# NyanCAD/Cadnip.jl

Hardware: AMD Instinct MI355X
Metric: newton_iters_per_sec (higher is better)
Workload: dtype f64; 1 GPU; gf180 DFF transient 0-700 ns (synthetic sp_mos1 level-1 card, 30 MOSFETs, n=235, nnz=1090), 4096 Vdd x temp corner instances per GPU (state resident in HBM; one 8-instance workgroup per CU in flight, the rest handed out by the kernel's instance queue); step = DC init + full transient of the batch; instances_per_gpu=4096, instances_total=4096, fused=2, newton_mode=1, launches_last_step=5120, accepted_last_step=6078488, rejected_last_step=692364

## Files before the change

### cadnip.jl_amd/csrc/devices.hpp

```cpp
#pragma once
#include <hip/hip_runtime.h>
#include <math.h>
#include "../../include/cadnip_hip.h"

namespace cadnip {

#define CADNIP_CHARGE_SCALE 1e12

#ifdef CADNIP_TRACE
static __device__ unsigned long long g_trace_sum[64], g_trace_cnt[64];
static __device__ int g_trace_wave;
__shared__ unsigned long long g_trace_last;
#define CADNIP_TRACE_FINE(id) (((id) >= 8 && (id) <= 15) || (id) >= 18 || (id) == 0 || (id) == 2)
#define CADNIP_TRACE_POINT(id)                                                                          \
  do {                                                                                                  \
    if ((CADNIP_TRACE + 0 >= 2 || !CADNIP_TRACE_FINE(id)) && blockIdx.x == 0 && (int)(threadIdx.x >> 6) == g_trace_wave) { \
      unsigned long long _t = clock64();                                                                \
      if ((threadIdx.x & 63) == 0) {                                                                    \
        atomicAdd(&g_trace_sum[id], _t - g_trace_last); atomicAdd(&g_trace_cnt[id], 1ull); g_trace_last = _t; \
      }                                                                                                 \
    }                                                                                                   \
  } while (0)
#define CADNIP_TRACE_USE(x) asm volatile("" ::"v"(x))
#elif defined(CADNIP_MARKS)
// ... 504 lines not shown
      D3 vddif = 2.0 * vdsat - vds, vddif1 = vdsat - vds, vddif2 = vddif * vddif;
      capgd = cox * (1.0 - vdsat * vdsat / vddif2) / 3;
      capgs = cox * (1.0 - vddif1 * vddif1 / vddif2) / 3;
      capgb = D3(0.0);
    }
  }
}

template <bool FQ = true>
__device__ inline D3 m1_qdep(const D3& v, double Cb, double Cbsw, double tBulkPot, double tDepCap, double mj, double mjsw,
                             double f2, double f3, double f4) {
  if (Cb != 0 || Cbsw != 0) {
    if (v.v < tDepCap) {
      D3 arg = 1.0 - m1_over<FQ>(v, tBulkPot);
      D3 sarg = (mj == 0.5) ? m1_recip<FQ>(m1_dsqrt<FQ>(arg)) : dexp(-mj * m1_dlog<FQ>(arg));
      D3 sargsw = (mjsw == mj) ? sarg : ((mjsw == 0.5) ? m1_recip<FQ>(m1_dsqrt<FQ>(arg)) : dexp(-mjsw * m1_dlog<FQ>(arg)));
      return tBulkPot * (m1_over<FQ>(Cb * (1.0 - arg * sarg), 1 - mj) + m1_over<FQ>(Cbsw * (1.0 - arg * sargsw), 1 - mjsw));
    }
    return f4 + v * (f2 + v * (f3 / 2));
  }
  return D3(0.0);
}

template <class Ctx>
__device__ inline void m1_limit(const Ctx& d, const double* u, double type, double vt, double tPhi, double tVbi, double gamma, double Vg, double Vb,
                                double Vdi, double Vsi, int l0, int l1, int l2, int l3, double& w_gs, double& w_ds, double& w_bs, double& w_bd) {
  double o_vgs = type * u[l0], o_vds = type * u[l1], o_vbs = type * u[l2], o_vbd = type * u[l3];
  double vbs = type * (Vb - Vsi), vgs = type * (Vg - Vsi), vds = type * (Vdi - Vsi);
  double vbd = vbs - vds, vgd = vgs - vds, vgdo = o_vgs - o_vds;
  {
    const bool fwd = o_vds >= 0;
    const double q_vgs = fwd ? vgs : vgd + (vgs - vgd), q_vgd = fwd ? vgs - (vgs - vgd) : vgd, q_vds = vgs - vgd;
    const bool c1 = fabs(fwd ? vgs - o_vgs : vgd - vgdo) <= 0.4, c2 = fabs(q_vds - o_vds) <= 0.4;
    const bool c3 = q_vds >= 0 ? !(fabs(vbs - o_vbs) > (vt + vt)) : !(fabs(vbd - o_vbd) > (vt + vt));
    if (__all(c1 && c2 && c3)) {
      double r_vgs = q_vgs, r_vds = q_vds, r_vbs, r_vbd;
      (void)q_vgd;
      if (r_vds >= 0) { r_vbs = vbs; r_vbd = r_vbs - r_vds; }
      else { r_vbd = vbd; r_vbs = r_vbd + r_vds; }
      if (d.initjct) { r_vbs = -1; r_vgs = type * par_of(d, M1_TVTO); r_vds = 0; r_vbd = r_vbs - r_vds; }
      w_gs = type * r_vgs; w_ds = type * r_vds; w_bs = type * r_vbs; w_bd = type * r_vbd;
      return;
    }
  }
  int omode = o_vds >= 0 ? 1 : -1;
  double osel = omode == 1 ? o_vbs : o_vbd, osarg;
  if (osel <= 0) osarg = sqrt(tPhi - osel);
  else { osarg = sqrt(tPhi); osarg = osarg - o_vbs / (osarg + osarg); osarg = fmax(0.0, osarg); }
  double o_von = (tVbi * type) + gamma * osarg;
  double von = type * o_von;
// ... 163 lines not shown
}


__device__ __forceinline__ D3 m1_swap_pair(const D3& x) {
  D3 r;
  r.v = dpp_pair_swap(x.v);
#pragma unroll
  for (int i = 0; i < 3; ++i) r.p[i] = dpp_pair_swap(x.p[i]);
  return r;
}
__device__ __forceinline__ D3 m1_sel(bool c, const D3& x, const D3& y) {
  D3 r;
  r.v = c ? x.v : y.v;
#pragma unroll
  for (int i = 0; i < 3; ++i) r.p[i] = c ? x.p[i] : y.p[i];
  return r;
}


template <class Ctx, class Out>
__device__ inline void stamp_mos1_pair(const Ctx& d, const double* u, const Out& s, double* limit_w_base, int side, bool valid) {
  const double CS = CADNIP_CHARGE_SCALE;
  const bool D = side != 0;
  int nd = node_of(d, 0), ng = node_of(d, 1), ns = node_of(d, 2), nb = node_of(d, 3), ndi = node_of(d, 4), nsi = node_of(d, 5);
  int l0 = node_of(d, 6), l1 = node_of(d, 7), l2 = node_of(d, 8), l3 = node_of(d, 9);
  double Vd = volt(u, nd), Vg = volt(u, ng), Vs = volt(u, ns), Vb = volt(u, nb), Vdi = volt(u, ndi), Vsi = volt(u, nsi);
  double type = par_of(d, M1_TYPE), vt = par_of(d, M1_VT), tPhi = par_of(d, M1_TPHI), tVbi = par_of(d, M1_TVBI);
  double gamma = par_of(d, M1_GAMMA);
  const double mf = par_of(d, M1_MFACTOR), gmin_p = par_of(d, M1_GMIN), isat = par_of(d, D ? M1_DSATCUR : M1_SSATCUR);
  const double lambda = par_of(d, M1_LAMBDA), Beta = par_of(d, M1_BETA);
  const int vdep = Out::DIRECT ? d.ipar[d.dev] : 0;
  __builtin_amdgcn_sched_barrier(0);
  CADNIP_TRACE_USE(Vd); CADNIP_TRACE_USE(Vg); CADNIP_TRACE_USE(Vs); CADNIP_TRACE_USE(Vb); CADNIP_TRACE_USE(Vdi); CADNIP_TRACE_USE(Vsi);
  CADNIP_TRACE_POINT(18);
  CADNIP_TRACE_USE(type);
  CADNIP_TRACE_POINT(19);
  CADNIP_TRACE_POINT(20);
  double w_gs, w_ds, w_bs, w_bd;
  m1_limit(d, u, type, vt, tPhi, tVbi, gamma, Vg, Vb, Vdi, Vsi, l0, l1, l2, l3, w_gs, w_ds, w_bs, w_bd);
  if (limit_w_base && valid && !D) { limit_w_base[l0] = w_gs; limit_w_base[l1] = w_ds; limit_w_base[l2] = w_bs; limit_w_base[l3] = w_bd; }
  CADNIP_TRACE_POINT(21);
  {
    const double gl[6] = {1.0, -1.0, 1.0, 1.0, -1.0, 1.0};
    s.Gv(6 * side, gl);
    if constexpr (Out::DIRECT) {
      s.Rn(D ? l2 : l0, u[D ? l2 : l0] - ((D ? Vb : Vg) - Vsi));
      s.Rn(D ? l3 : l1, u[D ? l3 : l1] - (D ? Vb - Vdi : Vdi - Vsi));
    }
  }
  CADNIP_TRACE_POINT(22);
  D3 a = D3::seed(type * w_gs, 0), b = D3::seed(type * w_ds, 1), c = D3::seed(type * w_bs, 2);
  D3 dvbd = c - b, dvgd = a - b;
  const D3 vj = m1_sel(D, dvbd, c);
  const double gmin_m = fast_div(gmin_p, mf);
  const double q_cb = par_of(d, D ? M1_CBD : M1_CBS), q_cbsw = par_of(d, D ? M1_CBDSW : M1_CBSSW), q_pot = par_of(d, M1_TBULKPOT), q_dep = par_of(d, M1_TDEPCAP);
  const double q_mj = par_of(d, M1_MJ), q_mjsw = par_of(d, M1_MJSW), q_f2 = par_of(d, D ? M1_F2D : M1_F2S), q_f3 = par_of(d, D ? M1_F3D : M1_F3S), q_f4 = par_of(d, D ? M1_F4D : M1_F4S);
  __builtin_amdgcn_sched_barrier(0);
  const D3 cj = m1_junction(vj, vt, gmin_m, isat), co = m1_swap_pair(cj);
  const D3 cbs = m1_sel(D, co, cj), cbd = m1_sel(D, cj, co);
  CADNIP_TRACE_POINT(23);
  int mode;
  D3 dvon, vdsat, cdrain;
  m1_channel(a, b, c, dvbd, dvgd, tPhi, tVbi, type, gamma, lambda, Beta, mode, dvon, vdsat, cdrain);
  CADNIP_TRACE_POINT(24);
  const D3 cdreq = (mode >= 0 ? type : -type) * cdrain;
  const double dW_gs = (Vg - Vsi) - w_gs, dW_ds = (Vdi - Vsi) - w_ds, dW_bs = (Vb - Vsi) - w_bs;
  const double Vk[6] = {Vd, Vg, Vs, Vb, Vdi, Vsi};
  auto row = [&](const D3& I, double (&g)[6], double& Ieq) {
    const double fa = type * I.p[0], fb = type * I.p[1], fc = type * I.p[2];
    g[0] = 0.0; g[1] = mf * fa; g[2] = 0.0; g[3] = mf * fc; g[4] = mf * fb; g[5] = mf * -(fa + fb + fc);
    Ieq = mf * I.v;
#pragma unroll
    for (int k = 0; k < 6; ++k) Ieq = Ieq + (-g[k] * Vk[k]);
    Ieq = Ieq + (mf * type * I.p[0]) * dW_gs;
    Ieq = Ieq + (mf * type * I.p[1]) * dW_ds;
    Ieq = Ieq + (mf * type * I.p[2]) * dW_bs;
  };
  {
    const D3 I3 = type * cbs + type * cbd, I4 = -1.0 * (type * cbd - cdreq);
    double g[6], Ieq;
    row(m1_sel(D, I4, I3), g, Ieq);
    const int br = 3 + side;
    s.Gv(12 + 6 * br, g);
    s.B(br, -Ieq);
    if constexpr (Out::DIRECT) {
      const D3 I = m1_sel(D, I4, I3);
      s.Rn(D ? ndi : nb, mf * I.v + (mf * type * I.p[0]) * dW_gs + (mf * type * I.p[1]) * dW_ds + (mf * type * I.p[2]) * dW_bs);
    }
  }
  {
    const D3 I5 = -1.0 * (cdreq + type * cbs);
    double g[6], Ieq;
    row(I5, g, Ieq);
    const int k2[2] = {12 + 30 + (D ? 4 : 1), 12 + 30 + (D ? 5 : 3)};
    const double v2[2] = {D ? g[4] : g[1], D ? g[5] : g[3]};
    s.Gk(k2, v2);
    if (Out::DIRECT || !D) s.B(5, -Ieq);
    if constexpr (Out::DIRECT)
      s.Rn(nsi, D ? 0.0 : mf * I5.v + (mf * type * I5.p[0]) * dW_gs + (mf * type * I5.p[1]) * dW_ds + (mf * type * I5.p[2]) * dW_bs);
  }
  CADNIP_TRACE_POINT(26);
  const D3 qj = m1_qdep(vj, q_cb, q_cbsw, q_pot, q_dep, q_mj, q_mjsw, q_f2, q_f3, q_f4);
  const D3 qo = m1_swap_pair(qj);
  const D3 qbs = m1_sel(D, qo, qj), qbd = m1_sel(D, qj, qo);
  CADNIP_TRACE_POINT(25);
  {
    const double cs2[2] = {1.0 / CS, 1.0 / CS};
    s.Cv(2 * side, cs2);
  }
  const D3 q0(0.0), q1 = type * qbs + type * qbd, q2 = -1.0 * (type * qbd), q3 = -1.0 * (type * qbs);
#pragma unroll
  for (int it = 0; it < 2; ++it) {
    const int r = 2 * it + side;
    const D3 q = it == 0 ? m1_sel(D, q1, q0) : m1_sel(D, q3, q2);
    const double fa = mf * type * q.p[0], fb = mf * type * q.p[1], fc = mf * type * q.p[2];
    const double dq[6] = {0.0, fa, 0.0, fc, fb, -(fa + fb + fc)};
    const double gq[7] = {1.0, -CS * dq[0], -CS * dq[1], -CS * dq[2], -CS * dq[3], -CS * dq[4], -CS * dq[5]};
    const bool cs_form = !Out::DIRECT || ((vdep >> r) & 1), lin_form = !Out::DIRECT || (!((vdep >> r) & 1) && r != 0);
    if (cs_form) s.Gv(48 + 7 * r, gq);
    double bc = mf * q.v;
#pragma unroll
    for (int k = 0; k < 6; ++k) bc -= dq[k] * Vk[k];
    bc += fa * dW_gs; bc += fb * dW_ds; bc += fc * dW_bs;
    s.B(6 + r, CS * bc);
    if (lin_form) s.Cv(4 + 6 * r, dq);
    if constexpr (Out::DIRECT) {
      const int np = r == 0 ? ng : r == 1 ? nb : r == 2 ? ndi : nsi;
      if ((vdep >> r) & 1) {
        const int nq = node_of(d, 10 + r);
        s.Rn(nq, u[nq] - CS * (mf * q.v + fa * dW_gs + fb * dW_ds + fc * dW_bs));
        s.Rn(np, s.du(nq) * (1.0 / CS));
      } else if (r != 0) {
        s.Rn(np, dq[1] * s.du(ng) + dq[3] * s.du(nb) + dq[4] * s.du(ndi) + dq[5] * s.du(nsi));
      }
    }
  }
  CADNIP_TRACE_POINT(27);
}

#define M1_NPAR 34
struct M1RegView {
  double p[M1_NPAR];
  int nd[14];
  int initjct;
};
__device__ __forceinline__ int node_of(const M1RegView& d, int k) { return d.nd[k]; }
__device__ __forceinline__ double par_of(const M1RegView& d, int k) { return d.p[k]; }
__device__ __forceinline__ double par_side(const M1RegView& d, int ks, int, bool) { return d.p[ks]; }
template <class Ctx> __device__ __forceinline__ double par_side(const Ctx& d, int ks, int kd, bool D) { return par_of(d, D ? kd : ks); }
__device__ __forceinline__ int node_side(const M1RegView& d, int ks, int kd, bool D) { return D ? d.nd[kd] : d.nd[ks]; }
template <class Ctx> __device__ __forceinline__ int node_side(const Ctx& d, int ks, int kd, bool D) { return node_of(d, D ? kd : ks); }
__device__ __forceinline__ void m1_load_params(M1RegView& v, const double* par, int count, int dev, bool D) {
#pragma unroll
  for (int k = 0; k < M1_NPAR; ++k) v.p[k] = par[k * count + dev];
  if (D) { v.p[M1_SSATCUR] = v.p[M1_DSATCUR]; v.p[M1_CBS] = v.p[M1_CBD]; v.p[M1_CBSSW] = v.p[M1_CBDSW]; v.p[M1_F2S] = v.p[M1_F2D]; v.p[M1_F3S] = v.p[M1_F3D]; v.p[M1_F4S] = v.p[M1_F4D]; }
}

#define M1_ROLE_J 1
#define M1_ROLE_Q 2
#define M1_ROLE_CH 4
template <class Ctx, class Out>
__device__ inline void stamp_mos1_team(const Ctx& d, const double* u, const Out& s, double* limit_w_base, int side, bool valid, int roles, int vdep) {
  static_assert(Out::DIRECT, "team stamping emits direct residuals");
  const double CS = CADNIP_CHARGE_SCALE;
  const bool D = side != 0;
  int ng = node_of(d, 1), nb = node_of(d, 3), ndi = node_of(d, 4), nsi = node_of(d, 5);
  int l0 = node_of(d, 6), l1 = node_of(d, 7), l2 = node_of(d, 8), l3 = node_of(d, 9);
  double Vg = volt(u, ng), Vb = volt(u, nb), Vdi = volt(u, ndi), Vsi = volt(u, nsi);
  double type = par_of(d, M1_TYPE), vt = par_of(d, M1_VT), tPhi = par_of(d, M1_TPHI), tVbi = par_of(d, M1_TVBI);
  double gamma = par_of(d, M1_GAMMA);
  const double mf = par_of(d, M1_MFACTOR);
  CADNIP_TRACE_POINT(20);
// ... 91 lines not shown
```

### cadnip.jl_amd/csrc/fused2.hip

```cpp
#include <hip/hip_runtime.h>
#include <stdio.h>
#include <stdlib.h>
#include <string.h>
#include <algorithm>
#include <vector>
#include "fused_team_kernel.hpp"

namespace cadnip {

struct F2Tables {
  std::vector<unsigned> data;
  int off[S_NSEC];
  void begin(int which) { if (data.size() & 1) data.push_back(0); off[which] = (int)data.size(); }
  void add16(const std::vector<int>& v) {
    for (size_t i = 0; i < v.size(); i += 2) data.push_back((unsigned)(v[i] & 0xFFFF) | ((i + 1 < v.size() ? (unsigned)(v[i + 1] & 0xFFFF) : 0u) << 16));
  }
  void add32(unsigned x) { data.push_back(x); }
  void add64(u64 x) { data.push_back((unsigned)x); data.push_back((unsigned)(x >> 32)); }
};

template <class Build>
static void upload_steps(StepList& L, int lu_words, Build&& build) {
  if (L.d) (void)hipFree(L.d);
  L = StepList();
// ... 212 lines not shown
  }
  if (mode == F2_STEP) return p;
  if (lean) p.steps = &S.steps1;
  auto bytes = [&](int wpb) { return lds_bytes(lds_sweep((size_t)0, p.tab_len, p.steps ? p.steps->len : 0, S.lu_words, h->n, 0, wpb)); };
  int wpb = 8;
  if (const char* e = getenv("CADNIP_F2_WPB")) wpb = atoi(e) >= 8 ? 8 : atoi(e) >= 4 ? 4 : atoi(e) >= 2 ? 2 : 1;
  while (wpb > 1 && (bytes(wpb) > LDS_BUDGET || S.n_cu * (wpb / 2) >= h->B)) wpb >>= 1;
  if (bytes(wpb) > LDS_BUDGET) return p;
  const int wg_per_cu = (int)std::max<size_t>(1, std::min<size_t>(LDS_BUDGET / bytes(wpb), (size_t)(32 / wpb)));
  size_t shmem = bytes(wpb);
  if (p.steps && lds_steps_predec_ok(S.lu_words, h->n) && !getenv("CADNIP_F2_STEPS_PACKED")) {
    const size_t pd = lds_bytes(lds_sweep((size_t)0, p.tab_len, lds_sweep_desc_words(p.steps->len, true), S.lu_words, h->n, 0, wpb));
    if (pd <= LDS_BUDGET && (int)std::max<size_t>(1, std::min<size_t>(LDS_BUDGET / pd, (size_t)(32 / wpb))) == wg_per_cu) { p.step_predec = true; shmem = pd; }
  }
  if (mode == F2_TRAN && direct && S.src_blk >= 0 && !env_is_zero("CADNIP_F2_SRC_CACHE")) {
    const int sw = src_cache_words(S.src_count), dw = p.steps ? lds_sweep_desc_words(p.steps->len, p.step_predec) : 0;
    if (src_cache_fits(p.tab_len, dw, S.lu_words, h->n, wpb, sw)) {
      p.src_words = sw;
      shmem = lds_bytes(lds_sweep((size_t)0, p.tab_len, dw, S.lu_words, h->n, 0, wpb, sw));
    }
  }
  p.fixed = topt && f2_fixed_ok(mode == F2_TRAN, p.var == 0, topt->newton_mode, p.step_predec, p.src_words, h->n, S.nc, topt->max_order, topt->step_rule,
                                topt->use_pcnr, !env_is_zero("CADNIP_F2_FIXED"));
  p.shape = f2_shape_ok(p.fixed, S.n_blk, S.src_type, S.src_count, S.rc_type, S.rc_count, S.dev_type, S.dev_plain, S.dev_count, !env_is_zero("CADNIP_F2_SHAPE"));
  p.wpb = wpb; p.shmem = shmem; p.grid = std::min((h->B + wpb - 1) / wpb, S.n_cu * wg_per_cu); p.rc = CADNIP_OK;
  return p;
}

static int launch_fused2(CadnipHandle* h, const TranArgs& t, int rounds, const F2DcOpts* dc, const F2StepOpts* step = nullptr) {
  const F2Plan p = fused2_plan(h, dc ? F2_DC : step ? F2_STEP : F2_TRAN, t.newton_mode, dc || step ? nullptr : &t);
  if (p.rc) return p.rc;
  ProfScope ps(h, dc ? "fused2_dc" : step ? "fused_step" : "fused2_newton");
  FusedState& S = h->f2;
  F2Args f{};
  f.n_blk = S.n_blk; f.rc_blk = S.rc_blk; f.src_blk = S.src_blk;
  f.blk = (const F2Block*)S.d_blk;
  f.wave = h->d_wave;
  f.tab = S.d_tab;
  for (int i = 0; i < S_NSEC; ++i) f.off[i] = S.off[i];
  f.tab_len = p.tab_len; f.tab_lo = p.tab_lo;
  f.n = h->n; f.nnz = h->nnz; f.nnz_lu = S.lu_words;
  f.n_pre = S.n_pre; f.n_post = S.n_post; f.nc = S.nc; f.dn0 = S.dn0; f.n_fwd = S.n_fwd;
  if (p.steps) { f.team_desc = p.steps->d; f.team_desc_len = p.steps->len; f.ts_pre = p.steps->n_steps[0]; f.ts_post = p.steps->n_steps[1]; f.ts_fwd = p.steps->n_steps[2]; }
  f.step_predec = p.step_predec ? 1 : 0;
  f.src_words = p.src_words;
  f.step_refresh = step ? step->refresh : 0; f.step_resid = step ? step->resid : nullptr; f.step_norm = step ? step->norm : nullptr;
  f.step_reps = step ? step->reps : 1; f.step_skip = step ? step->skip : 0;
// ... 54 lines not shown
```

### cadnip.jl_amd/csrc/fused2_kernel.hpp

```cpp
#pragma once
#include <hip/hip_runtime.h>
#include "devices.hpp"
#include "internal.hpp"
#include "tran_ctrl.hpp"
#include "lds_layout.hpp"
#include "src_cache.hpp"

namespace cadnip {

typedef unsigned short u16;
typedef unsigned long long u64;
#define NOPOS 0xFFFFu
#define F2_NCMAX 16
#define F2_JU 18
#define F2_MAX_BLOCKS 32

enum { S_GPOS = 0, S_CDESC, S_BROW, S_NZ, S_ENT, S_TERM, S_LEV, S_QINV, S_NODES, S_ROWOF, S_LOADPOS, S_NSEC };

struct F2Block {
  const int* ipar; const double* par;
  int type, count, n_par, g_base, c_base, b_base, nodes_off, mos1_plain;
  int lds_par;
};

// ... 55 lines not shown
  v.t = p->t.t; v.h = p->t.h; v.hprev = p->t.hprev; v.hpp = p->t.hpp; v.tcur = p->t.tcur; v.gamma = p->t.gamma;
  v.nhist = p->t.nhist; v.order = p->t.order; v.k = p->t.k; v.status = p->t.status; v.bp_idx = p->t.bp_idx; v.save_idx = p->t.save_idx;
  v.active = p->t.active; v.cnt = p->t.cnt; v.breaks = p->t.breaks; v.save_t = p->t.save_t; v.n_break = p->t.n_break; v.n_save = p->t.n_save;
  v.newton_mode = FIXED ? 1 : p->t.newton_mode; v.mn_a0f = p->t.mn_a0f; v.mn_ss = p->t.mn_ss; v.mn_dnp = p->t.mn_dnp; v.mn_flags = p->t.mn_flags;
  v.max_order = FIXED ? 2 : p->t.max_order; v.hp3 = FIXED ? nullptr : p->t.hp3;
  return v;
}

template <bool GUARD, bool DIRECT_, bool JAC = true>
struct AccumOutT {
  static constexpr bool DIRECT = DIRECT_;
  static_assert(JAC || DIRECT_, "a residual-only pass needs the direct residuals");
  double* W; const double* betas; double a0;
  const u16* gpos; const u64* cdesc; const u16* brow;
  int count, dev;
  unsigned sink;
  const double* us; const u16* rowof; unsigned trash;
  __device__ __forceinline__ unsigned tg(unsigned p) const { return GUARD && sink ? sink : p; }
  __device__ __forceinline__ double du(int node) const { return node < 0 ? 0.0 : a0 * us[node] + betas[node]; }
  __device__ __forceinline__ void Rn(int node, double v) const {
    if (!DIRECT) return;
    atomicAdd(&W[tg(node < 0 ? trash : (unsigned)rowof[node])], v);
  }
  __device__ __forceinline__ void G(int k, double v) const {
    if (!JAC) return;
    if (__builtin_constant_p(v) && v == 0.0) return;
    atomicAdd(&W[tg(gpos[k * count + dev])], v);
  }
  __device__ __forceinline__ void C(int k, double v) const {
    if (!JAC) return;
    if (__builtin_constant_p(v) && v == 0.0) return;
    const u64 d = cdesc[k * count + dev];
    atomicAdd(&W[tg((unsigned)d & 0xFFFFu)], a0 * v);
    if (!DIRECT) atomicAdd(&W[tg((unsigned)(d >> 16) & 0xFFFFu)], v * betas[(unsigned)(d >> 32) & 0xFFFFu]);
  }
  __device__ __forceinline__ void B(int k, double v) const {
    if (DIRECT || (__builtin_constant_p(v) && v == 0.0)) return;
    atomicAdd(&W[tg(brow[k * count + dev])], -v);
  }
  template <int N> __device__ __forceinline__ void Gv(int k0, const double (&v)[N]) const {
    if (!JAC) return;
    unsigned p[N];
#pragma unroll
    for (int i = 0; i < N; ++i) p[i] = gpos[(k0 + i) * count + dev];
#pragma unroll
    for (int i = 0; i < N; ++i) if (!(__builtin_constant_p(v[i]) && v[i] == 0.0)) atomicAdd(&W[tg(p[i])], v[i]);
// ... 14 lines not shown
    for (int i = 0; i < N; ++i) d[i] = cdesc[(k0 + i) * count + dev];
    if (!DIRECT) {
#pragma unroll
      for (int i = 0; i < N; ++i) bt[i] = betas[(unsigned)(d[i] >> 32) & 0xFFFFu];
    }
#pragma unroll
    for (int i = 0; i < N; ++i)
      if (!(__builtin_constant_p(v[i]) && v[i] == 0.0)) {
        atomicAdd(&W[tg((unsigned)d[i] & 0xFFFFu)], a0 * v[i]);
        if (!DIRECT) atomicAdd(&W[tg((unsigned)(d[i] >> 16) & 0xFFFFu)], v[i] * bt[i]);
      }
  }
  template <int N> __device__ __forceinline__ void Bv(int k0, const double (&v)[N]) const {
    if (DIRECT) return;
    unsigned p[N];
#pragma unroll
    for (int i = 0; i < N; ++i) p[i] = brow[(k0 + i) * count + dev];
#pragma unroll
    for (int i = 0; i < N; ++i) if (!(__builtin_constant_p(v[i]) && v[i] == 0.0)) atomicAdd(&W[tg(p[i])], -v[i]);
  }
};

typedef DevCtxT<short> LdsCtx;

template <bool LEAN, class Out>
__device__ __forceinline__ void dispatch_stamp2(int type, const LdsCtx& d, const double* u, const Out& s, double* lw) {
  if constexpr (LEAN) {
    switch (type) {
      case CADNIP_DEV_RESISTOR: stamp_resistor(d, u, s, lw); break;
      case CADNIP_DEV_CAPACITOR: stamp_capacitor(d, u, s, lw); break;
      case CADNIP_DEV_INDUCTOR: stamp_inductor(d, u, s, lw); break;
      case CADNIP_DEV_VSOURCE: stamp_vsource(d, u, s, lw); break;
      case CADNIP_DEV_ISOURCE: stamp_isource(d, u, s, lw); break;
      case CADNIP_DEV_VCVS: stamp_vcvs(d, u, s, lw); break;
      case CADNIP_DEV_VCCS: stamp_vccs(d, u, s, lw); break;
      case CADNIP_DEV_CCVS: stamp_ccvs(d, u, s, lw); break;
      case CADNIP_DEV_CCCS: stamp_cccs(d, u, s, lw); break;
    }
    return;
  }
  switch (type) {
    case CADNIP_DEV_RESISTOR: stamp_resistor(d, u, s, lw); break;
    case CADNIP_DEV_CAPACITOR: stamp_capacitor(d, u, s, lw); break;
    case CADNIP_DEV_INDUCTOR: stamp_inductor(d, u, s, lw); break;
    case CADNIP_DEV_VSOURCE: stamp_vsource(d, u, s, lw); break;
    case CADNIP_DEV_ISOURCE: stamp_isource(d, u, s, lw); break;
// ... 155 lines not shown
      for (int i = tid; i < f.team_desc_len; i += 64 * WPB) dst[i] = src[i];
    }
  }
  __syncthreads();
  const int nW = L.nW;
  double* W = L.W;
  double* us = L.u;
  double* betas = L.beta;
  if (lane0 == 0) { W[nW] = 0.0; W[nW + 1] = 1.0; }
  const int tlo = f.tab_lo;
  const u16* gpos = (const u16*)(tab + (f.off[S_GPOS] - tlo));
  const u64* cdesc = (const u64*)(tab + (f.off[S_CDESC] - tlo));
  const u16* brow = (const u16*)(tab + (f.off[S_BROW] - tlo));
  const u64* nzd = (const u64*)(tab + (LEAN ? 0 : f.off[S_NZ]));
  const u64* laned = (const u64*)(tab + (LEAN ? 0 : f.off[S_ENT]));
  const unsigned* term = tab + (LEAN ? 0 : f.off[S_TERM]);
  typedef const __attribute__((address_space(4))) u64* PassPtr;
  const PassPtr passd = (PassPtr)(const u64*)(f.tab + f.off[S_LEV]);
  const u16* qinv = (const u16*)(tab + (f.off[S_QINV] - tlo));
  const short* nodes = (const short*)(tab + (f.off[S_NODES] - tlo));
  const u16* rowof = (const u16*)(tab + (f.off[S_ROWOF] - tlo));
  unsigned rc_gp[RCQ][2] = {}, rc_row[RCQ] = {}, rc_nd[RCQ] = {}, src_gp[2] = {0, 0}, src_row[2] = {0, 0}, src_nd[2] = {0, 0};
  int rc_count = 0, rc_type = 0, src_count = 0, src_type = 0;
  if constexpr (DIRECT) {
    const unsigned tr = (unsigned)(f.nnz_lu + n + lane0);
    auto row_of = [&](int node) -> unsigned { return node < 0 ? tr : (unsigned)rowof[node]; };
    if (SHAPE ? true : f.rc_blk >= 0) {
      const F2Block B = load_block(f.blk, f.rc_blk);
      rc_count = B.count; rc_type = B.type;
      const short* nd = nodes + B.nodes_off;
#pragma unroll
      for (int q = 0; q < RCQ; ++q) {
        const int dev = lane0 + 64 * q;
        unsigned p[4] = {tr, tr, tr, tr};
        int np = -1, nn = -1;
        if (dev < B.count) {
          np = nd[dev]; nn = nd[B.count + dev];
#pragma unroll
          for (int k = 0; k < 4; ++k)
            p[k] = (SHAPE ? true : B.type == CADNIP_DEV_CAPACITOR) ? (unsigned)cdesc[B.c_base + k * B.count + dev] & 0xFFFFu : (unsigned)gpos[B.g_base + k * B.count + dev];
        }
        rc_gp[q][0] = p[0] | p[1] << 16; rc_gp[q][1] = p[2] | p[3] << 16;
        rc_row[q] = row_of(np) | row_of(nn) << 16;
        rc_nd[q] = ((unsigned)np & 0xFFFFu) | ((unsigned)nn & 0xFFFFu) << 16;
      }
    }
    if (SHAPE ? true : f.src_blk >= 0) {
      const F2Block B = load_block(f.blk, f.src_blk);
      src_count = B.count; src_type = B.type;
      const short* nd = nodes + B.nodes_off;
      unsigned p[4] = {tr, tr, tr, tr};
      int np = -1, nn = -1, ni = -1;
      if (lane0 < B.count) {
        np = nd[lane0]; nn = nd[B.count + lane0];
        if (SHAPE ? true : B.type == CADNIP_DEV_VSOURCE) {
          ni = nd[2 * B.count + lane0];
#pragma unroll
          for (int k = 0; k < 4; ++k) p[k] = (unsigned)gpos[B.g_base + k * B.count + lane0];
        }
      }
      src_gp[0] = p[0] | p[1] << 16; src_gp[1] = p[2] | p[3] << 16;
      src_row[0] = row_of(np) | row_of(nn) << 16; src_row[1] = row_of(ni);
      src_nd[0] = ((unsigned)np & 0xFFFFu) | ((unsigned)nn & 0xFFFFu) << 16; src_nd[1] = (unsigned)ni & 0xFFFFu;
    }
  }
#ifdef CADNIP_TRACE
  if (blockIdx.x == 0 && tid == 0) g_trace_last = clock64();
#endif
  int inst = blockIdx.x * WPB + w;
  int budget = f.rounds;
  for (;;) {
  StepState st;
  bool have = false;
  while (inst < f.B) {
    const TranStateView sv = state_view<FIXED>();
    if (DC) st.status = __builtin_amdgcn_readfirstlane(sv.status[inst]);
    else { st = load_state(sv, inst); make_uniform(st); }
    if (st.status == 0) { have = true; break; }
    int nx = 0;
    if (lane0 == 0) nx = atomicAdd(kargs()->queue, 1);
    inst = (int)gridDim.x * WPB + __builtin_amdgcn_readfirstlane(nx);
  }
  if (!have || budget <= 0) break;
  const size_t vo = (size_t)inst * n;
  double* lw = FIXED ? nullptr : (DC ? f.dc_pcnr : a.use_pcnr) ? kargs()->t.limit_w + vo : nullptr;
  FusedVecs<FIXED> vec{us, betas, W, qinv, vo, lw};
  if (!DC) vec.load_history(n, lane0);
  {
    const F2ArgsK ka = kargs();
    const double *ug = ka->t.u + vo, *betag = ka->t.beta + vo;
    for (int i = lane0; i < n; i += 64) { us[i] = ug[i]; betas[i] = DC ? 0.0 : betag[i]; }
  }
  const bool mn = FIXED ? true : !DC && LEAN && a.newton_mode != 0;
  if (mn && (st.mflags & MN_VALID)) {
    const double* src = kargs()->lufac + (size_t)inst * f.nnz_lu;
    for (int i = lane0; i < f.nnz_lu; i += 64) W[i] = src[i];
  }
  int dc_state = 0, dc_iters = 0, dc_first = 0;
  if (DC) { dc_state = __builtin_amdgcn_readfirstlane(kargs()->dcstate[inst]); dc_first = f.dc_initjct && __builtin_amdgcn_readfirstlane(kargs()->cold[inst]); }
  double rc_val[RCQ] = {};
  if (SHAPE ? true : f.rc_blk >= 0) {
    const F2Block B = load_block(f.blk, f.rc_blk);
    const double* par = B.par + (size_t)inst * B.n_par * B.count;
#pragma unroll
    for (int q = 0; q < RCQ; ++q) { const int dev = lane0 + 64 * q; rc_val[q] = par[dev < B.count ? dev : 0]; }
  }
  auto sc_on = [&]() -> bool { return FIXED ? true : !DC && DIRECT && kargs()->src_words > 0; };
  if (sc_on()) {
    const F2Block B = load_block(f.blk, f.src_blk);
    const int cl = src_cache_lanes(B.count);
    int ln = lane0;
    asm volatile("" : "+v"(ln));
    if (ln < cl) src_seg_store(L.src, cl, ln, src_seg_fill(B.ipar[ln], (B.par + (size_t)inst * B.n_par * B.count)[ln]));
  }
  double src_val = 0.0, src_t = 0.0;
  bool src_have = false;
  int src_seg = 0;
  for (; budget > 0; --budget) {
    int lane = lane0;
    asm volatile("" : "+v"(lane));
    CADNIP_TRACE_POINT(17);
    bool refresh = true;
    if (mn) {
      refresh = (st.mflags & MN_NEED) || !(st.mflags & MN_VALID) ||
                (st.k == 0 && (st.a0 < 0.6 * st.a0f || st.a0 * 0.6 > st.a0f || (st.mflags >> MN_SINCE_SHIFT) >= 20));
      if (refresh) { st.a0f = st.a0; st.ss = 20.0; st.mflags = MN_VALID | MN_JCUR; st.dsc = 1.0; }
      else st.dsc = st.a0 == st.a0f ? 1.0 : fast_div(2.0, 1.0 + fast_div(st.a0, st.a0f));
    }
// ... 68 lines not shown
            src_seg_store(L.src, cl, lane, r);
          }
          src_t = tcur; src_have = true;
        }
        CADNIP_TRACE_USE(src_val);
        CADNIP_TRACE_POINT(15);
        if (SHAPE ? true : src_type == CADNIP_DEV_VSOURCE) {
          const double ui = at(src_nd[1]), vd = at(src_nd[0] & 0xFFFFu) - at(src_nd[0] >> 16) - src_val;
          if (refresh) {
            atomicAdd(&W[src_gp[0] & 0xFFFFu], 1.0); atomicAdd(&W[src_gp[0] >> 16], -1.0);
            atomicAdd(&W[src_gp[1] & 0xFFFFu], 1.0); atomicAdd(&W[src_gp[1] >> 16], -1.0);
          }
          atomicAdd(&W[src_row[0] & 0xFFFFu], ui); atomicAdd(&W[src_row[0] >> 16], -ui);
          atomicAdd(&W[src_row[1]], vd);
        } else {
          atomicAdd(&W[src_row[0] & 0xFFFFu], -src_val); atomicAdd(&W[src_row[0] >> 16], src_val);
        }
      }
      CADNIP_TRACE_POINT(13);
    }
    if constexpr (SHAPE) {
      const int bi = 3 - f.rc_blk - f.src_blk;
      const F2Block B = load_block(f.blk, bi);
      const double* par = B.par + (size_t)inst * B.n_par * B.count;
      const int side = lane & 1;
      const int dv = lane >> 1;
      const bool valid = dv < B.count;
      LdsCtx d{nodes + B.nodes_off, B.ipar, par, f.wave, B.count, valid ? dv : B.count - 1, tcur, dmode, dinit};
      if (!refresh) {
        AccumOutT<true, DIRECT, false> s{W, betas, a0, gpos + B.g_base, cdesc + B.c_base, brow + B.b_base, B.count, d.dev, valid ? 0u : trash_w, us, rowof, trash_w};
        stamp_mos1_pair(d, us, s, lw, side, valid);
      } else {
        AccumOutT<true, DIRECT> s{W, betas, a0, gpos + B.g_base, cdesc + B.c_base, brow + B.b_base, B.count, d.dev, valid ? 0u : trash_w, us, rowof, trash_w};
        stamp_mos1_pair(d, us, s, lw, side, valid);
      }
      CADNIP_TRACE_POINT(8);
    }
    if constexpr (!SHAPE)
    for (int bi = 0; bi < f.n_blk; ++bi) {
      if (DIRECT && ((bi == f.rc_blk && rc_count <= 128) || (bi == f.src_blk && src_count <= 64))) continue;
      const F2Block B = load_block(f.blk, bi);
      const double* par = B.par + (size_t)inst * B.n_par * B.count;
      int dev0 = lane;
      if (DIRECT && bi == f.rc_blk) dev0 = lane + 128;
      if (DIRECT && bi == f.src_blk) dev0 = lane + 64;
      if (!DIRECT && bi == f.rc_blk) {
#pragma unroll
        for (int q = 0; q < 2; ++q) {
          const int dev = lane + 64 * q;
          if (dev < B.count) {
            AccumOutT<false, DIRECT> s{W, betas, a0, gpos + B.g_base, cdesc + B.c_base, brow + B.b_base, B.count, dev, 0u, us, rowof, trash_w};
            if (B.type == CADNIP_DEV_CAPACITOR) capacitance4(s, 0, rc_val[q]); else conductance4(s, 0, rc_val[q]);
            if (DIRECT) {
              const short* nd = nodes + B.nodes_off;
              const int np = nd[dev], nn = nd[B.count + dev];
              residual2(s, np, nn, B.type == CADNIP_DEV_CAPACITOR ? rc_val[q] * (s.du(np) - s.du(nn)) : rc_val[q] * (volt(us, np) - volt(us, nn)));
            }
// ... 285 lines not shown
```

### cadnip.jl_amd/csrc/lds_layout.hpp

```cpp
#pragma once
#include <stddef.h>
#include "../../include/cadnip_hip.h"
#ifdef __HIPCC__
#include <type_traits>
#define LDS_HD __host__ __device__ __forceinline__
#else
#define LDS_HD inline
#endif

#define F2_TRASH 64
#define LDS_BUDGET ((size_t)160 * 1024)
#define LDS_OPTIN ((size_t)64 * 1024)

namespace cadnip {

LDS_HD int lds_work_words(int lu_words, int n) { return lu_words + n + F2_TRASH; }
#define LDS_CONSTS 2

struct StepPredec { unsigned x, y, z, w, flags; };
LDS_HD StepPredec lds_step_predecode(unsigned x, unsigned y, unsigned z, unsigned w, unsigned trash_word) {
  StepPredec r;
  r.x = ((x & 0x8000u) ? (x & 0x7FFFu) : trash_word) << 3 | ((x >> 16) & 0x7FFFu) << 19;
  r.y = (y & 0x7FFF7FFFu) << 3; r.z = (z & 0x7FFF7FFFu) << 3; r.w = (w & 0x7FFF7FFFu) << 3;
  const unsigned lg = (x >> 31) | ((y >> 14) & 2u) | ((y >> 29) & 4u);
  const unsigned maxlg = ((z >> 15) & 1u) | ((z >> 30) & 2u) | ((w >> 13) & 4u);
  r.flags = lg << 4 | (w >> 31) << 3 | maxlg;
  return r;
}
LDS_HD bool lds_steps_predec_ok(int lu_words, int n) { return lu_words + n + F2_TRASH + LDS_CONSTS <= 8192; }
LDS_HD bool f2_fixed_ok(bool tran, bool lean, int newton_mode, bool step_predec, int src_words, int n, int nc, int max_order, int step_rule,
                        int use_pcnr, bool enabled) {
  return tran && lean && newton_mode == 1 && step_predec && src_words > 0 && n <= 256 && nc == 8 && max_order <= 2 && step_rule == 0 &&
         use_pcnr == 0 && enabled;
}
LDS_HD bool f2_shape_ok(bool fixed, int n_blk, int src_type, int src_count, int rc_type, int rc_count, int dev_type, int dev_plain, int dev_count,
                        bool enabled) {
  return fixed && n_blk == 3 && src_type == CADNIP_DEV_VSOURCE && src_count <= 64 && rc_type == CADNIP_DEV_CAPACITOR && rc_count <= 64 &&
         dev_type == CADNIP_DEV_MOS1 && dev_plain != 0 && dev_count <= 32 && enabled;
}
LDS_HD int lds_sweep_desc_words(int desc_len, bool predec) { return desc_len + (predec ? desc_len / 16 : 0); }

template <class P> struct LdsSweep { P desc, W, u, beta, end; int nW, per; P src; };
template <class P> LDS_HD LdsSweep<P> lds_sweep(P base, int tab_len, int desc_len, int lu_words, int n, int w, int wpb, int src_words = 0) {
  LdsSweep<P> L;
  L.nW = lds_work_words(lu_words, n);
  L.per = L.nW + LDS_CONSTS + 2 * n + src_words;
  L.desc = base + tab_len / 2;
  L.W = L.desc + desc_len + (size_t)w * L.per;
  L.u = L.W + L.nW + LDS_CONSTS; L.beta = L.u + n; L.src = L.beta + n;
  L.end = L.desc + desc_len + (size_t)wpb * L.per;
  return L;
}

template <class P> struct LdsTeam { P W, red, u, beta, par, desc, priv, end; int nW; };
template <class P> LDS_HD LdsTeam<P> lds_team(P base, int tab_len, int desc_len, int lu_words, int n, int par_words, int nw) {
  LdsTeam<P> L;
  L.nW = lds_work_words(lu_words, n);
  L.W = base + tab_len / 2;
  L.red = L.W + L.nW + LDS_CONSTS; L.u = L.red + 4 * nw; L.beta = L.u + n; L.par = L.beta + n;
  L.desc = L.par + ((par_words + 1) & ~1); L.priv = L.desc + desc_len;
  L.end = L.priv + (nw ? (size_t)(nw - 1) * L.nW : 0);
  return L;
// ... 48 lines not shown
```

Before: 169.9 million newton_iters/s.

## Pin MOS1 pair node offsets, rows and params in registers for shape kernel

Adds a register-resident MOS1 pair view for the fused shape path. Packed LDS byte offsets, residual row indices and the per-side device parameters are loaded once before the Newton loop, so each stamp no longer re-reads node tables, rowof and parameters from global or LDS memory. The stamp code is templated so the existing path is unchanged while the pinned view reads u and beta directly from LDS offsets. In exchange it raises VGPR pressure and adds an LDS-size guard that disables the shape path for large circuits.

```diff
diff --git a/cadnip.jl_amd/csrc/devices.hpp b/cadnip.jl_amd/csrc/devices.hpp
--- a/cadnip.jl_amd/csrc/devices.hpp
+++ b/cadnip.jl_amd/csrc/devices.hpp
@@ -550,10 +550,22 @@
   return D3(0.0);
 }
 
+enum { M1R_LA = 0, M1R_LB, M1R_ROW, M1R_SI, M1R_Q0, M1R_P0, M1R_Q1, M1R_P1 };
+template <class Ctx> struct m1_pinned { static constexpr bool value = false; };
+template <class Ctx> __device__ __forceinline__ double m1_ul(const Ctx&, const double* u, int l) { return u[l]; }
+template <class Ctx> __device__ __forceinline__ double m1_volt(const Ctx&, const double* u, int node) { return volt(u, node); }
+template <class Ctx, class Out> __device__ __forceinline__ double m1_du(const Ctx&, const Out& s, int node) { return s.du(node); }
+template <class Ctx, class Out> __device__ __forceinline__ void m1_Rn(const Ctx&, const Out& s, int, int node, double v) { s.Rn(node, v); }
+template <class Ctx> __device__ __forceinline__ int m1_vdep(const Ctx& d) { return d.ipar[d.dev]; }
+template <class Ctx> __device__ __forceinline__ int m1_qbit(const Ctx&, int vdep, int, int r) { return (vdep >> r) & 1; }
+template <class Ctx> __device__ __forceinline__ int m1_side(const Ctx&, int, int n_s, int n_d, bool D) { return D ? n_d : n_s; }
+template <class Ctx> __device__ __forceinline__ int m1_nq(const Ctx& d, int, int r) { return node_of(d, 10 + r); }
+template <class Ctx> __device__ __forceinline__ double par_side(const Ctx& d, int ks, int kd, bool D) { return par_of(d, D ? kd : ks); }
+
 template <class Ctx>
 __device__ inline void m1_limit(const Ctx& d, const double* u, double type, double vt, double tPhi, double tVbi, double gamma, double Vg, double Vb,
                                 double Vdi, double Vsi, int l0, int l1, int l2, int l3, double& w_gs, double& w_ds, double& w_bs, double& w_bd) {
-  double o_vgs = type * u[l0], o_vds = type * u[l1], o_vbs = type * u[l2], o_vbd = type * u[l3];
+  double o_vgs = type * m1_ul(d, u, l0), o_vds = type * m1_ul(d, u, l1), o_vbs = type * m1_ul(d, u, l2), o_vbd = type * m1_ul(d, u, l3);
   double vbs = type * (Vb - Vsi), vgs = type * (Vg - Vsi), vds = type * (Vdi - Vsi);
   double vbd = vbs - vds, vgd = vgs - vds, vgdo = o_vgs - o_vds;
   {
@@ -763,14 +775,15 @@
 __device__ inline void stamp_mos1_pair(const Ctx& d, const double* u, const Out& s, double* limit_w_base, int side, bool valid) {
   const double CS = CADNIP_CHARGE_SCALE;
   const bool D = side != 0;
+#define M1_PSIDE(ks, kd) (m1_pinned<Ctx>::value ? par_side(d, ks, kd, D) : par_of(d, D ? kd : ks))
   int nd = node_of(d, 0), ng = node_of(d, 1), ns = node_of(d, 2), nb = node_of(d, 3), ndi = node_of(d, 4), nsi = node_of(d, 5);
   int l0 = node_of(d, 6), l1 = node_of(d, 7), l2 = node_of(d, 8), l3 = node_of(d, 9);
-  double Vd = volt(u, nd), Vg = volt(u, ng), Vs = volt(u, ns), Vb = volt(u, nb), Vdi = volt(u, ndi), Vsi = volt(u, nsi);
+  double Vd = m1_volt(d, u, nd), Vg = m1_volt(d, u, ng), Vs = m1_volt(d, u, ns), Vb = m1_volt(d, u, nb), Vdi = m1_volt(d, u, ndi), Vsi = m1_volt(d, u, nsi);
   double type = par_of(d, M1_TYPE), vt = par_of(d, M1_VT), tPhi = par_of(d, M1_TPHI), tVbi = par_of(d, M1_TVBI);
   double gamma = par_of(d, M1_GAMMA);
-  const double mf = par_of(d, M1_MFACTOR), gmin_p = par_of(d, M1_GMIN), isat = par_of(d, D ? M1_DSATCUR : M1_SSATCUR);
+  const double mf = par_of(d, M1_MFACTOR), gmin_p = par_of(d, M1_GMIN), isat = M1_PSIDE(M1_SSATCUR, M1_DSATCUR);
   const double lambda = par_of(d, M1_LAMBDA), Beta = par_of(d, M1_BETA);
-  const int vdep = Out::DIRECT ? d.ipar[d.dev] : 0;
+  const int vdep = Out::DIRECT ? m1_vdep(d) : 0;
   __builtin_amdgcn_sched_barrier(0);
   CADNIP_TRACE_USE(Vd); CADNIP_TRACE_USE(Vg); CADNIP_TRACE_USE(Vs); CADNIP_TRACE_USE(Vb); CADNIP_TRACE_USE(Vdi); CADNIP_TRACE_USE(Vsi);
   CADNIP_TRACE_POINT(18);
@@ -779,14 +792,15 @@
   CADNIP_TRACE_POINT(20);
   double w_gs, w_ds, w_bs, w_bd;
   m1_limit(d, u, type, vt, tPhi, tVbi, gamma, Vg, Vb, Vdi, Vsi, l0, l1, l2, l3, w_gs, w_ds, w_bs, w_bd);
-  if (limit_w_base && valid && !D) { limit_w_base[l0] = w_gs; limit_w_base[l1] = w_ds; limit_w_base[l2] = w_bs; limit_w_base[l3] = w_bd; }
+  if constexpr (!m1_pinned<Ctx>::value)
+    if (limit_w_base && valid && !D) { limit_w_base[l0] = w_gs; limit_w_base[l1] = w_ds; limit_w_base[l2] = w_bs; limit_w_base[l3] = w_bd; }
   CADNIP_TRACE_POINT(21);
   {
     const double gl[6] = {1.0, -1.0, 1.0, 1.0, -1.0, 1.0};
     s.Gv(6 * side, gl);
     if constexpr (Out::DIRECT) {
-      s.Rn(D ? l2 : l0, u[D ? l2 : l0] - ((D ? Vb : Vg) - Vsi));
-      s.Rn(D ? l3 : l1, u[D ? l3 : l1] - (D ? Vb - Vdi : Vdi - Vsi));
+      m1_Rn(d, s, M1R_LA, m1_side(d, M1R_LA, l0, l2, D), m1_ul(d, u, m1_side(d, M1R_LA, l0, l2, D)) - ((D ? Vb : Vg) - Vsi));
+      m1_Rn(d, s, M1R_LB, m1_side(d, M1R_LB, l1, l3, D), m1_ul(d, u, m1_side(d, M1R_LB, l1, l3, D)) - (D ? Vb - Vdi : Vdi - Vsi));
     }
   }
   CADNIP_TRACE_POINT(22);
@@ -794,8 +808,8 @@
   D3 dvbd = c - b, dvgd = a - b;
   const D3 vj = m1_sel(D, dvbd, c);
   const double gmin_m = fast_div(gmin_p, mf);
-  const double q_cb = par_of(d, D ? M1_CBD : M1_CBS), q_cbsw = par_of(d, D ? M1_CBDSW : M1_CBSSW), q_pot = par_of(d, M1_TBULKPOT), q_dep = par_of(d, M1_TDEPCAP);
-  const double q_mj = par_of(d, M1_MJ), q_mjsw = par_of(d, M1_MJSW), q_f2 = par_of(d, D ? M1_F2D : M1_F2S), q_f3 = par_of(d, D ? M1_F3D : M1_F3S), q_f4 = par_of(d, D ? M1_F4D : M1_F4S);
+  const double q_cb = M1_PSIDE(M1_CBS, M1_CBD), q_cbsw = M1_PSIDE(M1_CBSSW, M1_CBDSW), q_pot = par_of(d, M1_TBULKPOT), q_dep = par_of(d, M1_TDEPCAP);
+  const double q_mj = par_of(d, M1_MJ), q_mjsw = par_of(d, M1_MJSW), q_f2 = M1_PSIDE(M1_F2S, M1_F2D), q_f3 = M1_PSIDE(M1_F3S, M1_F3D), q_f4 = M1_PSIDE(M1_F4S, M1_F4D);
   __builtin_amdgcn_sched_barrier(0);
   const D3 cj = m1_junction(vj, vt, gmin_m, isat), co = m1_swap_pair(cj);
   const D3 cbs = m1_sel(D, co, cj), cbd = m1_sel(D, cj, co);
@@ -826,7 +840,7 @@
     s.B(br, -Ieq);
     if constexpr (Out::DIRECT) {
       const D3 I = m1_sel(D, I4, I3);
-      s.Rn(D ? ndi : nb, mf * I.v + (mf * type * I.p[0]) * dW_gs + (mf * type * I.p[1]) * dW_ds + (mf * type * I.p[2]) * dW_bs);
+      m1_Rn(d, s, M1R_ROW, D ? ndi : nb, mf * I.v + (mf * type * I.p[0]) * dW_gs + (mf * type * I.p[1]) * dW_ds + (mf * type * I.p[2]) * dW_bs);
     }
   }
   {
@@ -838,7 +852,7 @@
     s.Gk(k2, v2);
     if (Out::DIRECT || !D) s.B(5, -Ieq);
     if constexpr (Out::DIRECT)
-      s.Rn(nsi, D ? 0.0 : mf * I5.v + (mf * type * I5.p[0]) * dW_gs + (mf * type * I5.p[1]) * dW_ds + (mf * type * I5.p[2]) * dW_bs);
+      m1_Rn(d, s, M1R_SI, nsi, D ? 0.0 : mf * I5.v + (mf * type * I5.p[0]) * dW_gs + (mf * type * I5.p[1]) * dW_ds + (mf * type * I5.p[2]) * dW_bs);
   }
   CADNIP_TRACE_POINT(26);
   const D3 qj = m1_qdep(vj, q_cb, q_cbsw, q_pot, q_dep, q_mj, q_mjsw, q_f2, q_f3, q_f4);
@@ -857,7 +871,7 @@
     const double fa = mf * type * q.p[0], fb = mf * type * q.p[1], fc = mf * type * q.p[2];
     const double dq[6] = {0.0, fa, 0.0, fc, fb, -(fa + fb + fc)};
     const double gq[7] = {1.0, -CS * dq[0], -CS * dq[1], -CS * dq[2], -CS * dq[3], -CS * dq[4], -CS * dq[5]};
-    const bool cs_form = !Out::DIRECT || ((vdep >> r) & 1), lin_form = !Out::DIRECT || (!((vdep >> r) & 1) && r != 0);
+    const bool cs_form = !Out::DIRECT || m1_qbit(d, vdep, it, r), lin_form = !Out::DIRECT || (!m1_qbit(d, vdep, it, r) && r != 0);
     if (cs_form) s.Gv(48 + 7 * r, gq);
     double bc = mf * q.v;
 #pragma unroll
@@ -867,16 +881,64 @@
     if (lin_form) s.Cv(4 + 6 * r, dq);
     if constexpr (Out::DIRECT) {
       const int np = r == 0 ? ng : r == 1 ? nb : r == 2 ? ndi : nsi;
-      if ((vdep >> r) & 1) {
-        const int nq = node_of(d, 10 + r);
-        s.Rn(nq, u[nq] - CS * (mf * q.v + fa * dW_gs + fb * dW_ds + fc * dW_bs));
-        s.Rn(np, s.du(nq) * (1.0 / CS));
+      if (m1_qbit(d, vdep, it, r)) {
+        const int nq = m1_nq(d, it, r);
+        m1_Rn(d, s, M1R_Q0 + 2 * it, nq, m1_ul(d, u, nq) - CS * (mf * q.v + fa * dW_gs + fb * dW_ds + fc * dW_bs));
+        m1_Rn(d, s, M1R_P0 + 2 * it, np, m1_du(d, s, nq) * (1.0 / CS));
       } else if (r != 0) {
-        s.Rn(np, dq[1] * s.du(ng) + dq[3] * s.du(nb) + dq[4] * s.du(ndi) + dq[5] * s.du(nsi));
+        m1_Rn(d, s, M1R_P0 + 2 * it, np, dq[1] * m1_du(d, s, ng) + dq[3] * m1_du(d, s, nb) + dq[4] * m1_du(d, s, ndi) + dq[5] * m1_du(d, s, nsi));
       }
     }
   }
+#undef M1_PSIDE
   CADNIP_TRACE_POINT(27);
+}
+
+template <class ParMem>
+struct M1PairView {
+  double p[M1_GMIN + 1];
+  unsigned opd[6];
+  unsigned row[4];
+  int initjct;
+  const double* W;
+  unsigned gnd, beta;
+  ParMem mem;
+};
+template <class M> struct m1_pinned<M1PairView<M>> { static constexpr bool value = true; };
+template <class M> __device__ __forceinline__ int m1_half(const M1PairView<M>&, const unsigned (&a)[6], int k) { return (int)((a[k >> 1] >> (16 * (k & 1))) & 0xFFFFu); }
+template <class M> __device__ __forceinline__ int node_of(const M1PairView<M>& d, int k) { return m1_half(d, d.opd, k); }
+template <class M> __device__ __forceinline__ double par_of(const M1PairView<M>& d, int k) {
+  return k == M1_TVTO || k == M1_SVCRIT || k == M1_DVCRIT ? d.mem(k) : d.p[k];
+}
+template <class M> __device__ __forceinline__ double par_side(const M1PairView<M>& d, int ks, int, bool) { return d.p[ks]; }
+template <class M> __device__ __forceinline__ int m1_vdep(const M1PairView<M>&) { return 0; }
+template <class M> __device__ __forceinline__ int m1_qbit(const M1PairView<M>& d, int, int it, int) { return (unsigned)m1_half(d, d.opd, 10 + it) != d.gnd; }
+template <class M> __device__ __forceinline__ int m1_side(const M1PairView<M>& d, int slot, int, int, bool D) { return D ? m1_half(d, d.opd, 8 + (slot - M1R_LA)) : m1_half(d, d.opd, 6 + (slot - M1R_LA)); }
+template <class M> __device__ __forceinline__ int m1_nq(const M1PairView<M>& d, int it, int) { return m1_half(d, d.opd, 10 + it); }
+template <class M> __device__ __forceinline__ double m1_ul(const M1PairView<M>& d, const double*, int off) { return *(const double*)((const char*)d.W + off); }
+template <class M> __device__ __forceinline__ double m1_volt(const M1PairView<M>& d, const double* u, int off) { return m1_ul(d, u, off); }
+template <class M, class Out> __device__ __forceinline__ double m1_du(const M1PairView<M>& d, const Out& s, int off) {
+  const double x = s.a0 * m1_ul(d, nullptr, off) + m1_ul(d, nullptr, off + (int)d.beta);
+  return (unsigned)off == d.gnd ? 0.0 : x;
+}
+template <class M, class Out> __device__ __forceinline__ void m1_Rn(const M1PairView<M>& d, const Out& s, int slot, int, double v) {
+  s.Rw((d.row[slot >> 1] >> (16 * (slot & 1))) & 0xFFFFu, v);
+}
+#define M1_PAIR_BOTH {M1_TYPE, M1_VT, M1_TPHI, M1_TVBI, M1_GAMMA, M1_MFACTOR, M1_GMIN, M1_LAMBDA, M1_BETA, M1_TBULKPOT, M1_TDEPCAP, M1_MJ, M1_MJSW}
+#define M1_PAIR_SIDED {{M1_SSATCUR, M1_DSATCUR}, {M1_CBS, M1_CBD}, {M1_CBSSW, M1_CBDSW}, {M1_F2S, M1_F2D}, {M1_F3S, M1_F3D}, {M1_F4S, M1_F4D}}
+template <class M> __device__ __forceinline__ void m1_pair_load_params(M1PairView<M>& v, const double* par, int count, int dev, bool D) {
+  constexpr int both[13] = M1_PAIR_BOTH, sided[6][2] = M1_PAIR_SIDED;
+#pragma unroll
+  for (int i = 0; i < 13; ++i) v.p[both[i]] = par[both[i] * count + dev];
+#pragma unroll
+  for (int i = 0; i < 6; ++i) v.p[sided[i][0]] = par[(D ? sided[i][1] : sided[i][0]) * count + dev];
+}
+template <class M, class F> __device__ __forceinline__ void m1_pair_each_param(M1PairView<M>& v, F&& fn) {
+  constexpr int both[13] = M1_PAIR_BOTH, sided[6][2] = M1_PAIR_SIDED;
+#pragma unroll
+  for (int i = 0; i < 13; ++i) fn(v.p[both[i]]);
+#pragma unroll
+  for (int i = 0; i < 6; ++i) fn(v.p[sided[i][0]]);
 }
 
 #define M1_NPAR 34
@@ -888,7 +950,6 @@
 __device__ __forceinline__ int node_of(const M1RegView& d, int k) { return d.nd[k]; }
 __device__ __forceinline__ double par_of(const M1RegView& d, int k) { return d.p[k]; }
 __device__ __forceinline__ double par_side(const M1RegView& d, int ks, int, bool) { return d.p[ks]; }
-template <class Ctx> __device__ __forceinline__ double par_side(const Ctx& d, int ks, int kd, bool D) { return par_of(d, D ? kd : ks); }
 __device__ __forceinline__ int node_side(const M1RegView& d, int ks, int kd, bool D) { return D ? d.nd[kd] : d.nd[ks]; }
 template <class Ctx> __device__ __forceinline__ int node_side(const Ctx& d, int ks, int kd, bool D) { return node_of(d, D ? kd : ks); }
 __device__ __forceinline__ void m1_load_params(M1RegView& v, const double* par, int count, int dev, bool D) {
diff --git a/cadnip.jl_amd/csrc/fused2.hip b/cadnip.jl_amd/csrc/fused2.hip
--- a/cadnip.jl_amd/csrc/fused2.hip
+++ b/cadnip.jl_amd/csrc/fused2.hip
@@ -258,7 +258,8 @@
   }
   p.fixed = topt && f2_fixed_ok(mode == F2_TRAN, p.var == 0, topt->newton_mode, p.step_predec, p.src_words, h->n, S.nc, topt->max_order, topt->step_rule,
                                 topt->use_pcnr, !env_is_zero("CADNIP_F2_FIXED"));
-  p.shape = f2_shape_ok(p.fixed, S.n_blk, S.src_type, S.src_count, S.rc_type, S.rc_count, S.dev_type, S.dev_plain, S.dev_count, !env_is_zero("CADNIP_F2_SHAPE"));
+  p.shape = f2_shape_ok(p.fixed, S.n_blk, S.src_type, S.src_count, S.rc_type, S.rc_count, S.dev_type, S.dev_plain, S.dev_count, !env_is_zero("CADNIP_F2_SHAPE")) &&
+            lds_m1pin_ok(S.lu_words, h->n);
   p.wpb = wpb; p.shmem = shmem; p.grid = std::min((h->B + wpb - 1) / wpb, S.n_cu * wg_per_cu); p.rc = CADNIP_OK;
   return p;
 }
diff --git a/cadnip.jl_amd/csrc/fused2_kernel.hpp b/cadnip.jl_amd/csrc/fused2_kernel.hpp
--- a/cadnip.jl_amd/csrc/fused2_kernel.hpp
+++ b/cadnip.jl_amd/csrc/fused2_kernel.hpp
@@ -101,6 +101,10 @@
     if (!DIRECT) return;
     atomicAdd(&W[tg(node < 0 ? trash : (unsigned)rowof[node])], v);
   }
+  __device__ __forceinline__ void Rw(unsigned word, double v) const {
+    if (!DIRECT) return;
+    atomicAdd(&W[tg(word)], v);
+  }
   __device__ __forceinline__ void G(int k, double v) const {
     if (!JAC) return;
     if (__builtin_constant_p(v) && v == 0.0) return;
@@ -161,6 +165,15 @@
 };
 
 typedef DevCtxT<short> LdsCtx;
+
+struct F2M1ParMem {
+  int bi, inst, dev;
+  __device__ __forceinline__ double operator()(int k) const {
+    const F2ArgsK ka = kargs();
+    const F2Block B = load_block(ka->blk, bi);
+    return (B.par + (size_t)inst * B.n_par * B.count)[k * B.count + dev];
+  }
+};
 
 template <bool LEAN, class Out>
 __device__ __forceinline__ void dispatch_stamp2(int type, const LdsCtx& d, const double* u, const Out& s, double* lw) {
@@ -362,6 +375,7 @@
   const u16* rowof = (const u16*)(tab + (f.off[S_ROWOF] - tlo));
   unsigned rc_gp[RCQ][2] = {}, rc_row[RCQ] = {}, rc_nd[RCQ] = {}, src_gp[2] = {0, 0}, src_row[2] = {0, 0}, src_nd[2] = {0, 0};
   int rc_count = 0, rc_type = 0, src_count = 0, src_type = 0;
+  M1PairView<F2M1ParMem> m1v;
   if constexpr (DIRECT) {
     const unsigned tr = (unsigned)(f.nnz_lu + n + lane0);
     auto row_of = [&](int node) -> unsigned { return node < 0 ? tr : (unsigned)rowof[node]; };
@@ -402,6 +416,25 @@
       src_gp[0] = p[0] | p[1] << 16; src_gp[1] = p[2] | p[3] << 16;
       src_row[0] = row_of(np) | row_of(nn) << 16; src_row[1] = row_of(ni);
       src_nd[0] = ((unsigned)np & 0xFFFFu) | ((unsigned)nn & 0xFFFFu) << 16; src_nd[1] = (unsigned)ni & 0xFFFFu;
+    }
+    if constexpr (SHAPE) {
+      const F2Block B = load_block(f.blk, 3 - f.rc_blk - f.src_blk);
+      const short* nd = nodes + B.nodes_off;
+      const int dv = lane0 >> 1, dev = dv < B.count ? dv : B.count - 1, sd = lane0 & 1;
+      const int vdep = B.ipar[dev];
+      auto node = [&](int k) -> int { return nd[k * B.count + dev]; };
+      auto qnode = [&](int r) -> int { return ((vdep >> r) & 1) ? node(10 + r) : -1; };
+      auto opd2 = [&](int na, int nb) -> unsigned { return lds_m1pin_operand(na, f.nnz_lu, n) | lds_m1pin_operand(nb, f.nnz_lu, n) << 16; };
+      auto row2 = [&](int na, int nb) -> unsigned { return lds_m1pin_row(rowof, na, tr) | lds_m1pin_row(rowof, nb, tr) << 16; };
+#pragma unroll
+      for (int j = 0; j < 5; ++j) m1v.opd[j] = opd2(node(2 * j), node(2 * j + 1));
+      m1v.opd[5] = opd2(qnode(sd), qnode(2 + sd));
+      m1v.row[0] = sd ? row2(node(8), node(9)) : row2(node(6), node(7));
+      m1v.row[1] = row2(sd ? node(4) : node(3), node(5));
+      m1v.row[2] = row2(qnode(sd), sd ? node(3) : node(1));
+      m1v.row[3] = row2(qnode(2 + sd), sd ? node(5) : node(4));
+      m1v.initjct = 0;
+      m1v.gnd = lds_m1pin_operand(-1, f.nnz_lu, n); m1v.beta = 8u * (unsigned)n;
     }
   }
 #ifdef CADNIP_TRACE
@@ -444,6 +477,11 @@
     const double* par = B.par + (size_t)inst * B.n_par * B.count;
 #pragma unroll
     for (int q = 0; q < RCQ; ++q) { const int dev = lane0 + 64 * q; rc_val[q] = par[dev < B.count ? dev : 0]; }
+  }
+  if constexpr (SHAPE) {
+    const F2Block B = load_block(f.blk, 3 - f.rc_blk - f.src_blk);
+    const int dv = lane0 >> 1;
+    m1_pair_load_params(m1v, B.par + (size_t)inst * B.n_par * B.count, B.count, dv < B.count ? dv : B.count - 1, (lane0 & 1) != 0);
   }
   auto sc_on = [&]() -> bool { return FIXED ? true : !DC && DIRECT && kargs()->src_words > 0; };
   if (sc_on()) {
@@ -558,17 +596,22 @@
     if constexpr (SHAPE) {
       const int bi = 3 - f.rc_blk - f.src_blk;
       const F2Block B = load_block(f.blk, bi);
-      const double* par = B.par + (size_t)inst * B.n_par * B.count;
       const int side = lane & 1;
       const int dv = lane >> 1;
       const bool valid = dv < B.count;
-      LdsCtx d{nodes + B.nodes_off, B.ipar, par, f.wave, B.count, valid ? dv : B.count - 1, tcur, dmode, dinit};
+      const int dev = valid ? dv : B.count - 1;
+#pragma unroll
+      for (int j = 0; j < 6; ++j) asm volatile("" : "+v"(m1v.opd[j]));
+#pragma unroll
+      for (int j = 0; j < 4; ++j) asm volatile("" : "+v"(m1v.row[j]));
+      m1_pair_each_param(m1v, [](double& x) { asm volatile("" : "+v"(x)); });
+      m1v.W = W; m1v.mem = F2M1ParMem{bi, inst, dev};
       if (!refresh) {
-        AccumOutT<true, DIRECT, false> s{W, betas, a0, gpos + B.g_base, cdesc + B.c_base, brow + B.b_base, B.count, d.dev, valid ? 0u : trash_w, us, rowof, trash_w};
-        stamp_mos1_pair(d, us, s, lw, side, valid);
+        AccumOutT<true, DIRECT, false> s{W, betas, a0, gpos + B.g_base, cdesc + B.c_base, brow + B.b_base, B.count, dev, valid ? 0u : trash_w, us, rowof, trash_w};
+        stamp_mos1_pair(m1v, us, s, lw, side, valid);
       } else {
-        AccumOutT<true, DIRECT> s{W, betas, a0, gpos + B.g_base, cdesc + B.c_base, brow + B.b_base, B.count, d.dev, valid ? 0u : trash_w, us, rowof, trash_w};
-        stamp_mos1_pair(d, us, s, lw, side, valid);
+        AccumOutT<true, DIRECT> s{W, betas, a0, gpos + B.g_base, cdesc + B.c_base, brow + B.b_base, B.count, dev, valid ? 0u : trash_w, us, rowof, trash_w};
+        stamp_mos1_pair(m1v, us, s, lw, side, valid);
       }
       CADNIP_TRACE_POINT(8);
     }
diff --git a/cadnip.jl_amd/csrc/lds_layout.hpp b/cadnip.jl_amd/csrc/lds_layout.hpp
--- a/cadnip.jl_amd/csrc/lds_layout.hpp
+++ b/cadnip.jl_amd/csrc/lds_layout.hpp
@@ -38,6 +38,12 @@
   return fixed && n_blk == 3 && src_type == CADNIP_DEV_VSOURCE && src_count <= 64 && rc_type == CADNIP_DEV_CAPACITOR && rc_count <= 64 &&
          dev_type == CADNIP_DEV_MOS1 && dev_plain != 0 && dev_count <= 32 && enabled;
 }
+LDS_HD bool lds_m1pin_ok(int lu_words, int n) { return lds_work_words(lu_words, n) + LDS_CONSTS + n <= 8192; }
+LDS_HD unsigned lds_m1pin_operand(int node, int lu_words, int n) {
+  const int nW = lds_work_words(lu_words, n);
+  return (unsigned)(node < 0 ? nW : nW + LDS_CONSTS + node) << 3;
+}
+template <class T> LDS_HD unsigned lds_m1pin_row(const T* rowof, int node, unsigned trash_word) { return node < 0 ? trash_word : (unsigned)rowof[node]; }
 LDS_HD int lds_sweep_desc_words(int desc_len, bool predec) { return desc_len + (predec ? desc_len / 16 : 0); }
 
 template <class P> struct LdsSweep { P desc, W, u, beta, end; int nW, per; P src; };
```

Measured after the change: 183.1 million newton_iters/s (median of 6 runs). 7.8% higher.
